# bluenote-1577/sylph

Hardware: AMD Instinct MI355X
Metric: read Gbp/s sketched + genome-comparisons/s profiled, 1 Gbp vs GTDB-R220 (higher is better)
Workload: dtype u64

## Files before the change

sylph_amd/csrc/device_common.h:

```cpp
#pragma once
#include <hip/hip_runtime.h>

#include <cstdint>

#include "seed_plan.h"

namespace sylph {

__device__ __forceinline__ uint64_t mm_hash64(uint64_t key) {
    key = ~(key + (key << 21));
    key = key ^ (key >> 24);
    key = (key + (key << 3)) + (key << 8);
    key = key ^ (key >> 14);
    key = (key + (key << 2)) + (key << 4);
    key = key ^ (key >> 28);
    key = key + (key << 31);
    return key;
}

template <int N>
__device__ __forceinline__ uint64_t lshl_add_u64(uint64_t a, uint64_t b) {
    uint64_t d;
    asm("v_lshl_add_u64 %0, %1, %2, %3" : "=v"(d) : "v"(a), "n"(N), "v"(b));
    return d;
}
template <uint32_t C>
__device__ __forceinline__ uint64_t mul_const_u64(uint64_t t) {
    uint32_t th;
    asm("v_mul_lo_u32 %0, %1, %2" : "=v"(th) : "v"((uint32_t)(t >> 32)), "s"(C));
    uint64_t d, carry;
    asm("v_mad_u64_u32 %0, %1, %2, %3, %4" : "=v"(d), "=s"(carry) : "v"((uint32_t)t), "s"(C - 1u), "v"(((uint64_t)th << 32) | (uint32_t)t));
    return d;
}
__device__ __forceinline__ uint64_t mm_hash64_gfx950(uint64_t key) {
    uint64_t t = lshl_add_u64<0>(key << 21, key);
    {
        uint64_t sh;
        asm("v_lshrrev_b64 %0, 24, %1" : "=v"(sh) : "v"(t));
        uint32_t hi;
        asm("v_bitop3_b32 %0, %1, %2, %3 bitop3:0x96" : "=v"(hi) : "v"((uint32_t)(t >> 32)), "v"((uint32_t)(sh >> 32)), "s"(0xFFFFFF00u));
        t = ((uint64_t)hi << 32) | ((uint32_t)t ^ (uint32_t)sh);
    }
    t = mul_const_u64<265>(t);
    t = t ^ (t >> 14);
    t = lshl_add_u64<4>(t, lshl_add_u64<2>(t, t));
    t = t ^ (t >> 28);
    t = lshl_add_u64<0>(t << 31, t);
    return t;
}
__device__ __forceinline__ uint32_t mm_hash64_gfx950_hi1(uint64_t key) {
    uint64_t t = lshl_add_u64<0>(key << 21, key);
    {
        uint64_t sh;
        asm("v_lshrrev_b64 %0, 24, %1" : "=v"(sh) : "v"(t));
        uint32_t hi;
        asm("v_bitop3_b32 %0, %1, %2, %3 bitop3:0x96" : "=v"(hi) : "v"((uint32_t)(t >> 32)), "v"((uint32_t)(sh >> 32)), "s"(0xFFFFFF00u));
        t = ((uint64_t)hi << 32) | ((uint32_t)t ^ (uint32_t)sh);
    }
    t = mul_const_u64<265>(t);
    t = t ^ (t >> 14);
    t = lshl_add_u64<4>(t, lshl_add_u64<2>(t, t));
    t = t ^ (t >> 28);
    return (uint32_t)(t >> 32) + __builtin_amdgcn_alignbit((uint32_t)(t >> 32), (uint32_t)t, 1) + 1u;
}

__device__ __forceinline__ uint64_t min_u62(uint64_t a, uint64_t b) { uint64_t d; asm("v_min_f64 %0, %1, %2" : "=v"(d) : "v"(a), "v"(b)); return d; }

template <int P>
__device__ __forceinline__ uint32_t fword(uint32_t A0, uint32_t A1, uint32_t A2) {
    static_assert(P >= 0 && P <= 64);
    if constexpr (P == 0) return A0;
    else if constexpr (P < 32) return __builtin_amdgcn_alignbit(A0, A1, 32 - P);
    else if constexpr (P == 32) return A1;
    else if constexpr (P < 64) return __builtin_amdgcn_alignbit(A1, A2, 64 - P);
    else return A2;
}
template <int Q>
__device__ __forceinline__ uint32_t rword(uint32_t B0, uint32_t B1, uint32_t B2) {
    static_assert(Q >= 0 && Q <= 64);
    if constexpr (Q == 0) return B0;
    else if constexpr (Q < 32) return __builtin_amdgcn_alignbit(B1, B0, Q);
    else if constexpr (Q == 32) return B1;
    else if constexpr (Q < 64) return __builtin_amdgcn_alignbit(B2, B1, Q - 32);
    else return B2;
}

__device__ __forceinline__ uint32_t byte_to_seq(uint32_t b) {
    const uint32_t u = b & 0xDFu;
    const uint32_t c = ((b >> 1) ^ (b >> 2)) & 3u;
    const bool acgtu = (u == 'A') | (u == 'C') | (u == 'G') | (u == 'T') | (u == 'U');
    return acgtu ? c : (b <= 3u ? b : 0u);
}

__device__ __forceinline__ uint32_t codes4_fast(uint32_t w, uint32_t& bad) {
    const uint32_t c = ((w >> 1) ^ (w >> 2)) & 0x03030303u;
    const uint32_t expect = __builtin_amdgcn_perm(0u, 0x54474341u , c);
    bad |= (w & 0xDFDFDFDFu) ^ expect;
    return c;
}
__device__ __forceinline__ uint32_t codes4_exact(uint32_t w) {
    return byte_to_seq(w & 0xFFu) | (byte_to_seq((w >> 8) & 0xFFu) << 8) | (byte_to_seq((w >> 16) & 0xFFu) << 16) |
           (byte_to_seq(w >> 24) << 24);
}

__device__ __forceinline__ uint32_t nonzero_bytes(uint32_t x) {
    return (((x & 0x7F7F7F7Fu) + 0x7F7F7F7Fu) | x) & 0x80808080u;
}
__device__ __forceinline__ void clear_invalid_codes(uint32_t w, uint32_t d, uint32_t& c, uint32_t& other) {
    const uint32_t inv = nonzero_bytes(d);
    const uint32_t not_u = nonzero_bytes((w & 0xDFDFDFDFu) ^ 0x55555555u), not_small = nonzero_bytes(w & 0xFCFCFCFCu);
    other |= inv & ~(not_u & not_small);
    c &= ~((inv >> 6) | (inv >> 7));
}

__device__ __forceinline__ uint32_t codes4_bitop(uint32_t w, uint32_t& diff) {
    uint32_t c;
    const uint32_t a = w >> 1, b = w >> 2, m = 0x03030303u, up = 0xDFDFDFDFu;
    asm("v_bitop3_b32 %0, %1, %2, %3 bitop3:0x28" : "=v"(c) : "v"(a), "v"(b), "v"(m));
    const uint32_t expect = __builtin_amdgcn_perm(0u, 0x54474341u , c);
    asm("v_bitop3_b32 %0, %1, %2, %3 bitop3:0x6a" : "=v"(diff) : "v"(w), "v"(up), "v"(expect));
    return c;
}
__device__ __forceinline__ uint32_t pack16_fwd(uint4 v) {
    uint32_t d0, d1, d2, d3, bad;
    uint32_t c0 = codes4_bitop(v.x, d0), c1 = codes4_bitop(v.y, d1), c2 = codes4_bitop(v.z, d2), c3 = codes4_bitop(v.w, d3);
    asm("v_or3_b32 %0, %1, %2, %3" : "=v"(bad) : "v"(d0), "v"(d1), "v"(d2));
    asm("v_or_b32 %0, %1, %2" : "=v"(bad) : "v"(bad), "v"(d3));
    if (bad) {
        uint32_t other = 0;
        clear_invalid_codes(v.x, d0, c0, other); clear_invalid_codes(v.y, d1, c1, other);
        clear_invalid_codes(v.z, d2, c2, other); clear_invalid_codes(v.w, d3, c3, other);
        if (other) { c0 = codes4_exact(v.x); c1 = codes4_exact(v.y); c2 = codes4_exact(v.z); c3 = codes4_exact(v.w); }
    }
    constexpr uint32_t GATHER = (1u << 30) | (1u << 20) | (1u << 10) | 1u;
    const uint32_t p0 = c0 * GATHER, p1 = c1 * GATHER, p2 = c2 * GATHER, p3 = c3 * GATHER;
    return __builtin_amdgcn_perm(p0, p1, 0x07030C0Cu) | __builtin_amdgcn_perm(p2, p3, 0x0C0C0703u);
}

__device__ __forceinline__ uint32_t rcword(uint32_t a) {
    const uint32_t r = __brev(a);
    return ~(((r & 0x55555555u) << 1) | ((r >> 1) & 0x55555555u));
}

__device__ __forceinline__ void pack16(uint4 v, uint32_t& F, uint32_t& R) {
    F = pack16_fwd(v);
    R = rcword(F);
}

using seed_plan::emission_rank;
using seed_plan::n_hashed_kmers;

__device__ __forceinline__ void wave_count_add(unsigned int* counter, bool pred) {
    const unsigned long long m = __ballot(pred);
    if (m && (__lane_id() == (unsigned)__ffsll((long long)m) - 1)) atomicAdd(counter, (unsigned int)__popcll(m));
}

__device__ __forceinline__ uint64_t find_record(const uint64_t* __restrict__ off, uint64_t n, uint64_t p) {
    uint64_t lo = 0, hi = n;
    while (hi - lo > 1) {
        const uint64_t mid = (lo + hi) >> 1;
        if (off[mid] <= p) lo = mid; else hi = mid;
    }
    return lo;
}

__device__ __forceinline__ uint32_t wave_inclusive_sum(uint32_t x) {
    x += (uint32_t)__builtin_amdgcn_update_dpp(0, (int)x, 0x111, 0xF, 0xF, false);
    x += (uint32_t)__builtin_amdgcn_update_dpp(0, (int)x, 0x112, 0xF, 0xF, false);
    x += (uint32_t)__builtin_amdgcn_update_dpp(0, (int)x, 0x114, 0xF, 0xF, false);
    x += (uint32_t)__builtin_amdgcn_update_dpp(0, (int)x, 0x118, 0xF, 0xF, false);
    x += (uint32_t)__builtin_amdgcn_update_dpp(0, (int)x, 0x142, 0xA, 0xF, false);
    x += (uint32_t)__builtin_amdgcn_update_dpp(0, (int)x, 0x143, 0xC, 0xF, false);
    return x;
}

__device__ __forceinline__ uint32_t wave_max_u32(uint32_t x) {
    x = max(x, (uint32_t)__builtin_amdgcn_update_dpp(0, (int)x, 0x111, 0xF, 0xF, false));
    x = max(x, (uint32_t)__builtin_amdgcn_update_dpp(0, (int)x, 0x112, 0xF, 0xF, false));
    x = max(x, (uint32_t)__builtin_amdgcn_update_dpp(0, (int)x, 0x114, 0xF, 0xF, false));
    x = max(x, (uint32_t)__builtin_amdgcn_update_dpp(0, (int)x, 0x118, 0xF, 0xF, false));
    x = max(x, (uint32_t)__builtin_amdgcn_update_dpp(0, (int)x, 0x142, 0xA, 0xF, false));
    x = max(x, (uint32_t)__builtin_amdgcn_update_dpp(0, (int)x, 0x143, 0xC, 0xF, false));
    return (uint32_t)__builtin_amdgcn_readlane((int)x, 63);
}

template <int TPB>
__device__ __forceinline__ uint32_t block_excl_sum(uint32_t v, uint32_t* s_wave, uint32_t* total) {
    const uint32_t lane = threadIdx.x & 63, wave = threadIdx.x >> 6;
    const uint32_t x = wave_inclusive_sum(v);
    __syncthreads();
    if (lane == 63) s_wave[wave] = x;
    __syncthreads();
    uint32_t base = 0, tot = 0;
#pragma unroll
    for (int w = 0; w < TPB / 64; w++) {
        const uint32_t t = s_wave[w];
        if ((uint32_t)w < wave) base += t;
        tot += t;
    }
    if (total) *total = tot;
    return base + x - v;
}

}
```

sylph_amd/csrc/position_road.hip:

```cpp
#include <algorithm>

#include "common.h"
#include "device_common.h"
#include "position_road.h"
#include "seeds.h"

namespace sylph {
namespace {

__device__ __forceinline__ void marker_halves(const uint8_t* __restrict__ p, uint32_t& even, uint32_t& odd) {
    uint32_t e = 0, o = 0;
    uint64_t xs[4];
    __builtin_memcpy(&xs[0], p, 16);
    __builtin_memcpy(&xs[2], p + 16, 16);
#pragma unroll
    for (int w = 0; w < 4; w++) {
        const uint64_t x = xs[w];
        uint32_t bad = 0;
        uint32_t lo = codes4_fast((uint32_t)x, bad), hi = codes4_fast((uint32_t)(x >> 32), bad);
        if (bad) { lo = codes4_exact((uint32_t)x); hi = codes4_exact((uint32_t)(x >> 32)); }
        const uint32_t ev = ((lo & 3u) << 6) | (((lo >> 16) & 3u) << 4) | ((hi & 3u) << 2) | ((hi >> 16) & 3u);
        const uint32_t od = (((lo >> 8) & 3u) << 6) | (((lo >> 24) & 3u) << 4) | (((hi >> 8) & 3u) << 2) | ((hi >> 24) & 3u);
        e = (e << 8) | ev;
        o = (o << 8) | od;
    }
    even = e;
    odd = o;
}

constexpr int COARSE_SHIFT = 14;
__global__ __launch_bounds__(256) void coarse_index_kernel(const uint64_t* __restrict__ off, uint64_t n_rec, uint32_t n_entries,
                                                           uint32_t* __restrict__ coarse) {
    const uint32_t t = blockIdx.x * blockDim.x + threadIdx.x;
    if (t >= n_entries) return;
    const uint64_t total = off[n_rec];
    uint64_t p = (uint64_t)t << COARSE_SHIFT;
    if (total == 0) { coarse[t] = 0; return; }
    if (p >= total) p = total - 1;
    coarse[t] = (uint32_t)find_record(off, n_rec, p);
}

template <bool LIGHT>
__global__ __launch_bounds__(256) void annotate_reads_kernel(
    const uint8_t* __restrict__ bases, const uint64_t* __restrict__ off, uint64_t n_rec, const uint32_t* __restrict__ pos, const uint64_t* __restrict__ hash,
    uint32_t n, uint32_t pos_bias, uint32_t k, int avx2_compat, int paired, int want_markers, uint64_t rec_base, const uint32_t* __restrict__ coarse,
    uint64_t* __restrict__ o_hash, OccRec* __restrict__ o_rec) {
    constexpr uint32_t WIN = 1024;
    __shared__ uint64_t s_lo, s_hi;
    __shared__ uint64_t s_off[WIN + 2];
    const uint32_t first = blockIdx.x * blockDim.x;
    const uint32_t i = first + threadIdx.x;
    const uint64_t total = off[n_rec];
    if (threadIdx.x == 0 || threadIdx.x == 64) {
        const uint32_t j = threadIdx.x == 0 ? first : min(n, first + blockDim.x) - 1;
        uint64_t p = pos[j] >= pos_bias ? pos[j] - pos_bias : 0;
        if (total && p >= total) p = total - 1;
        const uint64_t t = p >> COARSE_SHIFT;
        if (threadIdx.x == 0) s_lo = total ? coarse[t] : 0; else s_hi = (total ? coarse[t + 1] : 0) + 1;
    }
    __syncthreads();
    const uint64_t w_lo = s_lo & ~1ull;
    const uint64_t w_n = min(s_hi + 2, n_rec + 1) - w_lo;
    const bool in_lds = w_n <= WIN + 2;
    if (in_lds)
        for (uint32_t t = threadIdx.x; t < w_n; t += blockDim.x) s_off[t] = off[w_lo + t];
    __syncthreads();
    const bool live = i < n && pos[i] >= pos_bias;
    const uint64_t p = live ? pos[i] - pos_bias : ~0ull;
    uint64_t h = live ? hash[i] : 0, rid = 0, m0 = 0, m1 = 0;
    bool valid = false;
    if (p < total) {
        uint64_t r, start, L, s1 = 0, s2 = 0, e2 = 0;
        auto locate = [&](auto OFF) {
            uint64_t lo = s_lo, hi = s_hi;
            while (hi - lo > 1) {
                const uint64_t mid = (lo + hi) >> 1;
                if (OFF(mid) <= p) lo = mid; else hi = mid;
            }
            r = lo;
            start = OFF(r);
            L = OFF(r + 1) - start;
            if (paired) { const uint64_t r1 = r & ~1ull; s1 = OFF(r1); s2 = OFF(r1 + 1); e2 = OFF(r1 + 2); }
        };
        if (in_lds) locate([&](uint64_t q) -> uint64_t { return s_off[q - w_lo]; });
        else locate([&](uint64_t q) -> uint64_t { return off[q]; });
        valid = (p - start) < n_hashed_kmers(L, k, avx2_compat, 0);
        if (valid) {
            rid = rec_base + r;
            if (!LIGHT && want_markers) {
                const uint8_t* a = nullptr;
                const uint8_t* b = nullptr;
                if (!paired) {
                    if (L >= 66 && L <= 400) { a = bases + start; b = a + L / 2; }
                } else {
                    if (s2 - s1 >= 33 && e2 - s2 >= 33) { a = bases + s1; b = bases + s2; }
                }
                if (a) {
                    uint32_t f, g, rr, t;
                    marker_halves(a, f, g);
                    marker_halves(b, rr, t);
                    m0 = (uint64_t)f | ((uint64_t)rr << 32);
                    m1 = (uint64_t)g | ((uint64_t)t << 32);
                    rid |= RID_MARKER_BIT;
                    if (paired)
                        rid |= min(emission_rank((uint32_t)(p - start), (uint32_t)n_hashed_kmers(L, k, avx2_compat, 0), avx2_compat), RID_RANK_MAX)
                               << RID_RANK_SHIFT;
                }
            }
        }
    }
    if (i < n) {
        const uint64_t hv = valid ? h : INVALID_HASH;
        o_hash[i] = hv;
        if constexpr (!LIGHT) o_rec[i] = OccRec{hv, rid, m0, m1};
    }
}

__global__ __launch_bounds__(256) void annotate_contigs_kernel(const uint64_t* __restrict__ off, uint64_t n_contigs, const uint32_t* __restrict__ pos,
                                                               const uint64_t* __restrict__ hash, uint32_t n, uint32_t k, int avx2_compat,
                                                               uint32_t* __restrict__ o_contig, uint64_t* __restrict__ o_pos, uint64_t* __restrict__ o_hash) {
    const uint32_t i = blockIdx.x * blockDim.x + threadIdx.x;
    if (i >= n) return;
    const uint64_t p = pos[i];
    uint64_t h = INVALID_HASH, endpos = 0;
    uint32_t contig = 0;
    if (p < off[n_contigs]) {
        const uint64_t r = find_record(off, n_contigs, p);
        const uint64_t start = off[r], L = off[r + 1] - start;
        if ((p - start) < n_hashed_kmers(L, k, avx2_compat, 1)) {
            h = hash[i];
            contig = (uint32_t)r;
            endpos = p - start + k - 1;
        }
    }
    o_contig[i] = contig;
    o_pos[i] = endpos;
    o_hash[i] = h;
}

}

PosSeeds seeds_sorted_by_pos(sylph_ctx* ctx, const uint8_t* d_bases, uint64_t n_bases, uint32_t c, uint32_t k, uint32_t* d_count) {
    SY_REQUIRE(n_bases < (1ull << 32), "a batch may hold at most 2^32-1 bases (got %llu)", (unsigned long long)n_bases);
    const PosSeeds none{nullptr, nullptr, 0};
    if (n_bases == 0) return none;
    DevBuf &b_pos = ctx->scratch[2], &b_hash = ctx->scratch[3];
    if (ctx->seeds_mode != 1) {
        HostPhase ph(ctx, "push: seeds (ordered slots)");
        const uint32_t n_tiles = seeds_n_tiles(n_bases), slot_cap = seeds_slot_capacity(c);
        DevBuf &b_sh = ctx->scratch[0], &b_sp = ctx->scratch[1], &b_tc = ctx->scratch[4];
        b_sh.reserve((size_t)n_tiles * slot_cap * 8);
        b_sp.reserve((size_t)n_tiles * slot_cap * 4);
        b_tc.reserve(((size_t)n_tiles + 1) * 4 * 3 + sizeof(SpillState) + 16);
        uint32_t* tile_count = b_tc.as<uint32_t>();
        uint32_t* tile_off = tile_count + (n_tiles + 1);
        uint32_t* spill_slot = tile_off + (n_tiles + 1);
        SpillState* d_spill = reinterpret_cast<SpillState*>(spill_slot + n_tiles + 1);
        SY_HIP(hipMemsetAsync(tile_count + n_tiles, 0, 4, ctx->stream));
        SY_HIP(hipMemsetAsync(d_spill, 0, 4, ctx->stream));
        launch_seeds_slots(ctx, d_bases, (uint32_t)n_bases, c, k, slot_cap, b_sh.as<uint64_t>(), b_sp.as<uint32_t>(), tile_count, d_spill, nullptr, 0, nullptr);
        exclusive_sum_u32(ctx, tile_count, tile_off, (size_t)n_tiles + 1);
        uint32_t res[2] = {0, 0};
        SY_HIP(hipMemcpyAsync(ctx->pinned, tile_off + n_tiles, 4, hipMemcpyDeviceToHost, ctx->stream));
        SY_HIP(hipMemcpyAsync((uint8_t*)ctx->pinned + 4, d_spill, 4, hipMemcpyDeviceToHost, ctx->stream));
        SY_HIP(hipStreamSynchronize(ctx->stream));
        memcpy(res, ctx->pinned, 8);
        if (!ctx->pending.empty()) profile_collect(ctx);
        if (res[1] <= SPILL_MAX_TILES) {
            if (res[0] == 0) return none;
            uint64_t* xh = nullptr;
            uint32_t* xp = nullptr;
            if (res[1]) {
                DevBuf& b_x = ctx->scratch[7];
                const size_t tb = seeds_tile_bases();
                b_x.reserve((size_t)res[1] * tb * 12);
                xh = b_x.as<uint64_t>();
                xp = reinterpret_cast<uint32_t*>(xh + (size_t)res[1] * tb);
                ScopedKernelTimer ts(ctx, "seeds_spill");
                launch_seeds_slots(ctx, d_bases, (uint32_t)n_bases, c, k, slot_cap, xh, xp, tile_count, d_spill, d_spill->tiles, res[1], spill_slot);
            }
            b_pos.reserve((size_t)res[0] * 4);
            b_hash.reserve((size_t)res[0] * 8);
            launch_compact_slots(ctx, b_sh.as<uint64_t>(), b_sp.as<uint32_t>(), tile_count, tile_off, n_tiles, slot_cap, xh, xp, spill_slot,
                                 b_pos.as<uint32_t>(), b_hash.as<uint64_t>());
            return PosSeeds{b_pos.as<uint32_t>(), b_hash.as<uint64_t>(), res[0]};
        }
    }
    uint64_t cap = n_bases / c + n_bases / (4ull * c) + 65536;
    if (cap > n_bases) cap = n_bases;
    uint32_t n = 0;
    for (int attempt = 0; attempt < 2; attempt++) {
        HostPhase ph(ctx, "push: seeds kernel");
        ctx->scratch[0].reserve(cap * 8);
        ctx->scratch[1].reserve(cap * 4);
        static const bool slowlog = getenv("SYLPH_HIP_SLOWLOG") != nullptr;
        const double t0 = slowlog ? HostPhase::now() : 0;
        SY_HIP(hipMemsetAsync(d_count, 0, 4, ctx->stream));
        const double t1 = slowlog ? HostPhase::now() : 0;
        if (slowlog && t1 - t0 > 3.0) fprintf(stderr, "[sylph_hip] slow memset issue %.3f ms\n", t1 - t0);
        launch_seeds(ctx, d_bases, (uint32_t)n_bases, c, k, ctx->scratch[0].as<uint64_t>(), ctx->scratch[1].as<uint32_t>(), (uint32_t)cap, d_count);
        ctx->read_back(&n, d_count, 4);
        if (n <= cap) break;
        cap = n;
        SY_REQUIRE(attempt == 0, "seed buffer overflow persisted");
    }
    if (n == 0) return none;
    HostPhase ph(ctx, "push: sort by position");
    b_pos.reserve((size_t)n * 4);
    b_hash.reserve((size_t)n * 8);
    sort_pairs_u32_u64(ctx, ctx->scratch[1].as<uint32_t>(), b_pos.as<uint32_t>(), ctx->scratch[0].as<uint64_t>(), b_hash.as<uint64_t>(), n, 0,
                       std::max(1, bit_length(n_bases)));
    return PosSeeds{b_pos.as<uint32_t>(), b_hash.as<uint64_t>(), n};
}

void annotate_reads(sylph_sketch* sk, const uint8_t* d_bases, const uint64_t* d_off, uint64_t n_records, uint64_t n_bases, uint32_t bias,
                    const PosSeeds& s, bool plain) {
    sylph_ctx* ctx = sk->ctx;
    const uint32_t n_coarse = (uint32_t)(n_bases >> COARSE_SHIFT) + 2;
    DevBuf& b_coarse = ctx->scratch[5];
    b_coarse.reserve((size_t)n_coarse * 4);
    ScopedKernelTimer t(ctx, "annotate");
    hipLaunchKernelGGL(coarse_index_kernel, dim3(grid_for64(n_coarse)), dim3(256), 0, ctx->stream, d_off, n_records, n_coarse, b_coarse.as<uint32_t>());
    auto annotate = [&](auto kernel, int want_markers, OccRec* o_rec) {
        hipLaunchKernelGGL(kernel, dim3(grid_for64(s.n)), dim3(256), 0, ctx->stream, d_bases, d_off, n_records, s.pos, s.hash, s.n, bias, sk->k, sk->avx2_compat,
                           sk->paired, want_markers, sk->rec_base, b_coarse.as<uint32_t>(), sk->hash.as<uint64_t>() + sk->n_occ, o_rec);
    };
    if (plain) annotate(annotate_reads_kernel<true>, 0, nullptr);
    else annotate(annotate_reads_kernel<false>, sk->no_dedup ? 0 : 1, sk->recs.as<OccRec>() + sk->n_occ);
    SY_HIP(hipGetLastError());
}


struct ContigSeeds { std::vector<uint32_t> contig; std::vector<uint64_t> pos, hash; };

static void seeds_positions_impl(sylph_ctx* ctx, const uint8_t* bases, const uint64_t* contig_off, uint64_t n_contigs, uint32_t c, uint32_t k, int seed_mode, ContigSeeds& out) {
    SY_REQUIRE(c >= 1, "c must be >= 1");
    SY_REQUIRE(seed_mode == SYLPH_SEED_SCALAR || seed_mode == SYLPH_SEED_AVX2_COMPAT, "bad seed_mode %d", seed_mode);
    SY_REQUIRE(k == 21 || k == 31, "k must be 21 or 31 (avx2_seeding.rs:46-52)");
    if (n_contigs == 0) return;
    SY_REQUIRE(contig_off && contig_off[0] == 0, "bad contig offsets");
    SY_REQUIRE(bases || contig_off[n_contigs] == 0, "null bases");
    SY_REQUIRE(n_contigs < (1ull << 32), "too many contigs");
    std::lock_guard<std::mutex> lock(ctx->mu);
    DeviceGuard dg(ctx->device);
    const uint64_t n_bases = contig_off[n_contigs];
    SY_REQUIRE(n_bases < (1ull << 32), "genome larger than 2^32-1 bases: split by contig");
    DevBuf d_bases(ctx), d_off(ctx);
    d_bases.reserve(n_bases + 64);
    d_off.reserve((n_contigs + 1) * 8);
    ctx->h2d(d_bases.p, bases, n_bases);
    ctx->h2d(d_off.p, contig_off, (n_contigs + 1) * 8);
    ctx->counters.reserve(64);
    const PosSeeds s = seeds_sorted_by_pos(ctx, d_bases.as<uint8_t>(), n_bases, c, k, ctx->counters.as<uint32_t>());
    const uint32_t n = s.n;
    if (!n) return;
    DevBuf o_contig(ctx), o_pos(ctx), o_hash(ctx);
    o_contig.reserve((size_t)n * 4);
    o_pos.reserve((size_t)n * 8);
    o_hash.reserve((size_t)n * 8);
    {
        ScopedKernelTimer t(ctx, "annotate");
        hipLaunchKernelGGL(annotate_contigs_kernel, dim3(grid_for64(n)), dim3(256), 0, ctx->stream, d_off.as<uint64_t>(), n_contigs, s.pos, s.hash, n, k,
                           seed_mode == SYLPH_SEED_AVX2_COMPAT, o_contig.as<uint32_t>(), o_pos.as<uint64_t>(), o_hash.as<uint64_t>());
        SY_HIP(hipGetLastError());
    }
    std::vector<uint32_t> hc(n);
    std::vector<uint64_t> hp(n), hh(n);
    ctx->d2h(hc.data(), o_contig.p, (size_t)n * 4);
    ctx->d2h(hp.data(), o_pos.p, (size_t)n * 8);
    ctx->d2h(hh.data(), o_hash.p, (size_t)n * 8);
    out.contig.reserve(n); out.pos.reserve(n); out.hash.reserve(n);
    for (uint32_t i = 0; i < n; i++) {
        if (hh[i] == INVALID_HASH) continue;
        out.contig.push_back(hc[i]); out.pos.push_back(hp[i]); out.hash.push_back(hh[i]);
    }
}

template <class T>
static T* to_malloc(const std::vector<T>& v) {
    T* p = (T*)malloc(std::max<size_t>(1, v.size()) * sizeof(T));
    if (!p) throw std::bad_alloc();
    if (!v.empty()) memcpy(p, v.data(), v.size() * sizeof(T));
    return p;
}

}

using namespace sylph;

extern "C" {

int sylph_seeds_positions(sylph_ctx* ctx, const uint8_t* bases, const uint64_t* contig_off, uint64_t n_contigs, uint32_t c,
                          uint32_t k, int seed_mode, uint32_t** out_contig, uint64_t** out_pos, uint64_t** out_hash,
                          uint64_t* out_n) {
    return guarded([&] {
        SY_REQUIRE(ctx && out_contig && out_pos && out_hash && out_n, "null argument");
        ContigSeeds s;
        seeds_positions_impl(ctx, bases, contig_off, n_contigs, c, k, seed_mode, s);
        *out_contig = to_malloc(s.contig);
        *out_pos = to_malloc(s.pos);
        *out_hash = to_malloc(s.hash);
        *out_n = s.hash.size();
    });
}

int sylph_seeds(sylph_ctx* ctx, const uint8_t* bases, uint64_t len, uint32_t c, uint32_t k, int seed_mode,
                uint64_t** out_hashes, uint64_t* out_n) {
    return guarded([&] {
        SY_REQUIRE(ctx && out_hashes && out_n, "null argument");
        SY_REQUIRE(c >= 1, "c must be >= 1");
        SY_REQUIRE(k == 21 || k == 31, "k must be 21 or 31 (avx2_seeding.rs:46-52)");
        SY_REQUIRE(seed_mode == SYLPH_SEED_SCALAR || seed_mode == SYLPH_SEED_AVX2_COMPAT, "bad seed_mode %d", seed_mode);
        std::vector<uint64_t> res;
        if (len) {
            SY_REQUIRE(bases, "null bases");
            SY_REQUIRE(len < (1ull << 32), "sequence longer than 2^32-1 bases");
            std::lock_guard<std::mutex> lock(ctx->mu);
            DeviceGuard dg(ctx->device);
            DevBuf d_bases(ctx);
            d_bases.reserve(len + 64);
            ctx->h2d(d_bases.p, bases, len);
            ctx->counters.reserve(64);
            const PosSeeds s = seeds_sorted_by_pos(ctx, d_bases.as<uint8_t>(), len, c, k, ctx->counters.as<uint32_t>());
            if (const uint32_t n = s.n) {
                std::vector<uint32_t> hp(n);
                std::vector<uint64_t> hh(n);
                ctx->d2h(hp.data(), s.pos, (size_t)n * 4);
                ctx->d2h(hh.data(), s.hash, (size_t)n * 8);
                const uint64_t nk = n_hashed_kmers(len, k, seed_mode == SYLPH_SEED_AVX2_COMPAT, 0);
                for (uint32_t i = 0; i < n; i++)
                    if (hp[i] < nk) res.push_back(hh[i]);
            }
        }
        *out_hashes = to_malloc(res);
        *out_n = res.size();
    });
}

}
```

sylph_amd/csrc/reads_block.h:

```cpp
#pragma once
#include "common.h"
#include "device_common.h"
#include "seed_plan.h"
#include "sketch_session.h"

namespace sylph {
namespace {

using namespace seed_plan;

template <int K>
struct KC {
    static constexpr uint64_t MASK = (1ull << (2 * K)) - 1;
};

#define SY_LDS __attribute__((address_space(3)))
template <int TPB>
struct ReadsLds {
    SY_LDS uint32_t* sF;
    SY_LDS uint64_t* off;
    SY_LDS uint64_t *m0, *m1;
    SY_LDS uint32_t (*mask)[TPB];
    SY_LDS uint32_t* wave;
    SY_LDS uint32_t* first;
    SY_LDS uint32_t* hist;
    SY_LDS uint32_t* rel;
    SY_LDS uint16_t *perm, *nh;
    SY_LDS uint32_t *redo, *redo_deal;
};
template <int TPB>
__device__ __forceinline__ ReadsLds<TPB> reads_lds() {
    constexpr int OFFS = offs_staged(TPB);
    extern __shared__ uint32_t sF[];
    __shared__ uint64_t s_off[OFFS + 4];
    __shared__ uint32_t s_mask[MASKW][TPB];
    __shared__ uint32_t s_wave[TPB / 64];
    __shared__ uint32_t s_first[TPB + 1], s_rel[TPB];
    __shared__ uint16_t s_perm[TPB], s_nh[TPB];
    __shared__ uint32_t s_redo, s_redo_deal;
    static_assert((OFFS + 4) >= 2 * TPB, "the marker arrays alias the staged offsets");
    static_assert(TPB + 1 >= 64, "the histogram aliases s_first");
    using W = SY_LDS uint32_t*; using D = SY_LDS uint64_t*; using H = SY_LDS uint16_t*;
    return ReadsLds<TPB>{(W)sF, (D)s_off, (D)s_off, (D)s_off + TPB, (SY_LDS uint32_t(*)[TPB])s_mask, (W)s_wave, (W)s_first, (W)s_first, (W)s_rel,
                         (H)s_perm, (H)s_nh, (W)&s_redo, (W)&s_redo_deal};
}

__device__ __forceinline__ uint64_t win64(const SY_LDS uint32_t* sF, uint32_t b) {
    const uint32_t j = b >> 4, ph = (b & 15u) * 2u;
    const uint64_t x = ((uint64_t)sF[j] << 32) | sF[j + 1];
    return (x << ph) | ((uint64_t)sF[j + 2] >> (32u - ph));
}

template <int K>
__device__ __forceinline__ uint64_t revcomp_top(uint64_t x) {
    const uint64_t rev = __brevll(x);
    const uint64_t y = ((rev & 0x5555555555555555ull) << 1) | ((rev >> 1) & 0x5555555555555555ull);
    return (~y) & KC<K>::MASK;
}

__device__ __forceinline__ uint32_t even_fields_to_bytes31(uint32_t w) {
    uint32_t t = w & 0xCCCCCCCCu;
    t = (t | (t << 2)) & 0xF0F0F0F0u;
    return t | (t << 4);
}
__device__ __forceinline__ void evenodd16(uint64_t x, uint32_t& ev, uint32_t& od) {
    const uint32_t hi = (uint32_t)(x >> 32), lo = (uint32_t)x;
    ev = __builtin_amdgcn_perm(even_fields_to_bytes31(hi), even_fields_to_bytes31(lo), 0x07050301u);
    od = __builtin_amdgcn_perm(even_fields_to_bytes31(hi << 2), even_fields_to_bytes31(lo << 2), 0x07050301u);
}

struct HitRegs {
    uint32_t bit[16];
    uint32_t zero;
    uint64_t exec0;
};
__device__ __forceinline__ HitRegs hit_regs() {
    HitRegs r;
#pragma unroll
    for (int t = 0; t < 16; t++) asm("v_mov_b32 %0, %1" : "=v"(r.bit[t]) : "s"(hit_const(t)));
    asm("v_mov_b32 %0, 0" : "=v"(r.zero));
    r.exec0 = 0;
    return r;
}
__device__ __forceinline__ void hit_clear_lower(uint32_t& addr, uint32_t zero) { asm("ds_write_b16 %0, %1" : "+v"(addr) : "v"(zero)); }
__device__ __forceinline__ void hit_chain_begin(uint32_t& addr) { asm volatile("" : "+v"(addr) : : "memory"); }
__device__ __forceinline__ void hit_chain_end(uint32_t& addr) { asm volatile("s_waitcnt lgkmcnt(0)" : "+v"(addr) : : "memory"); }

template <int K, int T, int HV, bool LB>
__device__ __forceinline__ void kmer_step(uint32_t A0, uint32_t A1, uint32_t A2, uint32_t B0, uint32_t B1, uint32_t B2,
                                          uint64_t thr, uint32_t& mask, const HitRegs& hit) {
    static_assert(2 * K <= 62 && 2 * K > 32, "min_u62 wants both windows below 2^62; the high word holds 2K - 32 bits");
    constexpr int HB = 2 * K - 32, T0 = T & ~1;
    uint32_t fhi, rhi;
    if constexpr (2 * T + HB <= 32) {
        fhi = __builtin_amdgcn_ubfe(A0, 32 - HB - 2 * T, HB); rhi = __builtin_amdgcn_ubfe(B1, 2 * T, HB);
    } else {
        const uint32_t cf = fword<2 * T0>(A0, A1, A2), cr = rword<2 * T0 + 32>(B0, B1, B2);
        fhi = __builtin_amdgcn_ubfe(cf, 32 - HB - 2 * (T - T0), HB); rhi = __builtin_amdgcn_ubfe(cr, 2 * (T - T0), HB);
    }
    const uint32_t flo = fword<2 * T + HB>(A0, A1, A2), rlo = rword<2 * T>(B0, B1, B2);
    const uint64_t canon = min_u62(((uint64_t)fhi << 32) | flo, ((uint64_t)rhi << 32) | rlo);
    if constexpr (HV == 2) {
        const uint32_t u = mm_hash64_gfx950_hi1(canon);
        if constexpr (LB)
            asm("v_cmpx_ge_u32 vcc, %2, %1\n\tds_xor_b32 %0, %3\n\ts_mov_b64 exec, %4"
                : "+v"(mask) : "v"(u), "s"((uint32_t)thr), "v"(hit.bit[T]), "s"(hit.exec0) : "vcc");
        else
            asm("v_cmp_ge_u32 vcc, %2, %1\n\tv_addc_co_u32 %0, vcc, %0, %0, vcc" : "+v"(mask) : "v"(u), "s"((uint32_t)thr) : "vcc");
    } else {
        const uint64_t h = HV ? mm_hash64_gfx950(canon) : mm_hash64(canon);
        if constexpr (LB)
            asm("v_cmpx_lt_u64 vcc, %1, %2\n\tds_xor_b32 %0, %3\n\ts_mov_b64 exec, %4"
                : "+v"(mask) : "v"(h), "s"(thr), "v"(hit.bit[T]), "s"(hit.exec0) : "vcc");
        else
            asm("v_cmp_lt_u64 vcc, %1, %2\n\tv_addc_co_u32 %0, vcc, %0, %0, vcc" : "+v"(mask) : "v"(h), "s"(thr) : "vcc");
    }
}
template <int K, int T0, int HV, bool LB>
__device__ __forceinline__ void kmer_steps8(uint32_t A0, uint32_t A1, uint32_t A2, uint32_t B0, uint32_t B1, uint32_t B2,
                                            uint64_t thr, uint32_t& mask, const HitRegs& hit) {
    kmer_step<K, T0 + 0, HV, LB>(A0, A1, A2, B0, B1, B2, thr, mask, hit);
    kmer_step<K, T0 + 1, HV, LB>(A0, A1, A2, B0, B1, B2, thr, mask, hit);
    kmer_step<K, T0 + 2, HV, LB>(A0, A1, A2, B0, B1, B2, thr, mask, hit);
    kmer_step<K, T0 + 3, HV, LB>(A0, A1, A2, B0, B1, B2, thr, mask, hit);
    kmer_step<K, T0 + 4, HV, LB>(A0, A1, A2, B0, B1, B2, thr, mask, hit);
    kmer_step<K, T0 + 5, HV, LB>(A0, A1, A2, B0, B1, B2, thr, mask, hit);
    kmer_step<K, T0 + 6, HV, LB>(A0, A1, A2, B0, B1, B2, thr, mask, hit);
    kmer_step<K, T0 + 7, HV, LB>(A0, A1, A2, B0, B1, B2, thr, mask, hit);
}

template <int ENC, int TPB>
__device__ __forceinline__ void load_stream(SY_LDS uint32_t* sF, const uint8_t* bases_al, uint64_t n_al, uint32_t blk, int64_t a0, uint32_t n_words) {
    const uint32_t tid = threadIdx.x;
    const bool interior = block_starts_inside(blk) && (uint64_t)(a0 + (int64_t)n_words * 16) <= n_al;
    const uintptr_t src0 = (uintptr_t)bases_al + (uintptr_t)(ENC == 0 ? a0 : (a0 >> 2));
    constexpr uint32_t WB = ENC == 0 ? 16u : 4u;
    if (interior) {
        if constexpr (ENC == 0) {
            for (uint32_t ci = tid; ci < n_words; ci += TPB) sF[ci] = pack16_fwd(*reinterpret_cast<const uint4*>(src0 + ci * WB));
        } else {
            for (uint32_t ci = tid; ci < n_words; ci += TPB)
                sF[ci] = __builtin_amdgcn_perm(0u, *reinterpret_cast<const uint32_t*>(src0 + ci * WB), 0x00010203u);
        }
    } else {
        uint32_t ci_lo, ci_hi;
        stream_word_range(a0, n_al, n_words, ci_lo, ci_hi);
        for (uint32_t ci = tid; ci < n_words; ci += TPB) {
            const bool inside = ci >= ci_lo && ci < ci_hi;
            if constexpr (ENC == 0) {
                uint4 v = make_uint4(0, 0, 0, 0);
                if (inside) v = *reinterpret_cast<const uint4*>(src0 + ci * WB);
                sF[ci] = pack16_fwd(v);
            } else {
                uint32_t w = 0;
                if (inside) w = *reinterpret_cast<const uint32_t*>(src0 + ci * WB);
                sF[ci] = __builtin_amdgcn_perm(0u, w, 0x00010203u);
            }
        }
    }
}

template <int TPB>
__device__ __forceinline__ bool stage_offsets(const ReadsLds<TPB> s, const uint64_t* off, uint64_t n_rec, uint32_t R0, uint32_t R1,
                                              uint32_t w_lo) {
    const uint32_t w_hi = R1 + min((uint32_t)n_rec - R1, 2u);
    const uint32_t n_stage = w_hi - w_lo + 1;
    const bool in_lds = n_stage <= (uint32_t)(offs_staged(TPB) + 4) && (R1 - R0) <= (uint32_t)TPB;
    if (in_lds) {
        const uint64_t* const src = off + w_lo;
        for (uint32_t t = threadIdx.x; t < n_stage; t += TPB) s.off[t] = src[t];
    }
    return in_lds;
}

template <int K, int TPB>
__device__ __forceinline__ bool record_geometry(const ReadsLds<TPB> s, const uint64_t* off, bool in_lds, uint32_t w_lo, uint32_t r,
                                                bool active, int paired, uint32_t rb, int avx2_compat, int want_markers, uint32_t& nh,
                                                uint32_t& rel, uint32_t& ba, uint32_t& bb) {
    uint64_t o0 = 0, o1 = 0, o2 = 0;
    if (active) {
        const uint32_t r0 = paired ? (r & ~1u) : r;
        if (in_lds) {
            const SY_LDS uint64_t* const o = s.off + (r0 - w_lo);
            o0 = o[0]; o1 = o[1];
            if (paired) o2 = o[2];
        } else {
            const uint64_t* const o = off + r0;
            o0 = o[0]; o1 = o[1];
            if (paired) o2 = o[2];
        }
    }
    const uint64_t d1 = o1 - o0, d2 = o2 - o1;
    const bool too_long = d1 > (uint64_t)RH || (paired && d2 > (uint64_t)RH);
    const bool mate2 = paired && (r & 1u);
    const uint32_t L = too_long ? 0u : (uint32_t)(mate2 ? d2 : d1);
    const uint32_t rel1 = record_rel32(o0, rb), rel2 = record_rel32(o1, rb);
    nh = (uint32_t)n_hashed_kmers(L, K, avx2_compat, 0);
    rel = active ? (mate2 ? rel2 : rel1) : 0u;
    MarkerBases mk{0u, 0u};
    if (want_markers && active && !too_long) mk = paired ? pair_marker_bases(rel1, rel2, (uint32_t)d1, (uint32_t)d2) : single_marker_bases(rel, L);
    ba = mk.ba; bb = mk.bb;
    return too_long;
}

template <int TPB, bool LB>
__device__ __forceinline__ bool deal_by_length(const ReadsLds<TPB> s, uint32_t nh, uint32_t rel, uint32_t& slot, uint32_t& rel_h, uint32_t& nh_h,
                                               uint32_t& rows) {
    const uint32_t tid = threadIdx.x, lane = tid & 63;
    if (tid < 64) s.hist[tid] = 0;
    s.rel[tid] = rel;
    s.nh[tid] = (uint16_t)nh;
    if (tid == 0) *s.redo_deal = 0;
    __syncthreads();
    if (__ballot(nh != (uint32_t)s.nh[0]) && lane == 0) *s.redo_deal = 1;
    __syncthreads();
    const bool dealt = *s.redo_deal != 0;
    const uint32_t bin = deal_bin(nh);
    uint32_t hg_max = half_groups(nh), arrival = 0, hc = 0;
    if (dealt) {
        arrival = atomicAdd((uint32_t*)&s.hist[bin], 1u);
        __syncthreads();
        hc = s.hist[lane];
        const uint64_t bins_used = __ballot(hc != 0u);
        hg_max = bins_used ? 63u - (uint32_t)(__ffsll((unsigned long long)bins_used) - 1) : 0u;
    }
    rows = rows_used(hg_max);
    if constexpr (LB) {
        const uint32_t rows_u = (uint32_t)__builtin_amdgcn_readfirstlane((int)rows);
        for (uint32_t w = 0; w < rows_u; w += 2) { s.mask[w][tid] = 0; s.mask[w + 1][tid] = 0; }
    }
    if (dealt) {
        const uint32_t incl = wave_inclusive_sum(hc);
        s.perm[(uint32_t)__shfl((int)(incl - hc), (int)bin) + arrival] = (uint16_t)tid;
        __syncthreads();
    }
    slot = dealt ? s.perm[tid] : tid;
    rel_h = dealt ? s.rel[slot] : rel;
    nh_h = dealt ? s.nh[slot] : nh;
    return dealt;
}

template <int K, int HV, int TPB, bool LB>
__device__ __forceinline__ void hash_record(const ReadsLds<TPB> s, uint32_t slot, uint32_t rel_h, uint32_t nh_h, uint64_t thr_loop,
                                            const HitRegs& hit_consts) {
    const SY_LDS uint32_t* const sF = s.sF;
    const uint32_t nh_max = wave_max_u32(nh_h);
    if (nh_max) {
        const uint32_t w0 = rel_h >> 4, sh = 32u - (rel_h & 15u) * 2u;
        uint32_t raw = sF[w0], nxt = sF[w0 + 1];
        auto next_word = [&](uint32_t j) {
            const uint32_t a = (uint32_t)((((uint64_t)raw << 32) | nxt) >> sh);
            raw = nxt;
            nxt = sF[w0 + j + 2];
            return a;
        };
        uint32_t A0 = next_word(0), A1 = next_word(1), A2 = next_word(2);
        uint32_t B0 = rcword(A0), B1 = rcword(A1), B2 = rcword(A2);
        const uint32_t n_half = half_groups(nh_max);
        SY_LDS uint16_t* const mask_half = (SY_LDS uint16_t*)&s.mask[0][slot];
        const uint32_t n_grp = n_half >> 1;
        if constexpr (LB) {
            HitRegs hit = hit_consts;
            hit.exec0 = __builtin_amdgcn_read_exec();
            uint32_t addr = (uint32_t)(uintptr_t)&s.mask[0][slot];
            hit_chain_begin(addr);
            for (uint32_t g = 0; g < n_grp; g++) {
                kmer_steps8<K, 0, HV, true>(A0, A1, A2, B0, B1, B2, thr_loop, addr, hit);
                kmer_steps8<K, 8, HV, true>(A0, A1, A2, B0, B1, B2, thr_loop, addr, hit);
                A0 = A1; A1 = A2; A2 = next_word(g + 3);
                B0 = B1; B1 = B2; B2 = rcword(A2);
                if (hit_clear_after(g)) hit_clear_lower(addr, hit.zero);
                else addr += hit_word_offset(2, TPB);
            }
            if (n_half & 1u) {
                kmer_steps8<K, 0, HV, true>(A0, A1, A2, B0, B1, B2, thr_loop, addr, hit);
                if (hit_clear_after(n_grp)) hit_clear_lower(addr, hit.zero);
            }
            hit_chain_end(addr);
            return;
        }
        const HitRegs hit{};
        for (uint32_t g = 0; g < n_grp; g++) {
            uint32_t mask = 0;
            kmer_steps8<K, 0, HV, false>(A0, A1, A2, B0, B1, B2, thr_loop, mask, hit);
            kmer_steps8<K, 8, HV, false>(A0, A1, A2, B0, B1, B2, thr_loop, mask, hit);
            A0 = A1; A1 = A2; A2 = next_word(g + 3);
            B0 = B1; B1 = B2; B2 = rcword(A2);
            mask_half[group_half(g, TPB)] = (uint16_t)mask;
        }
        if (n_half & 1u) {
            uint32_t mask = 0;
            kmer_steps8<K, 0, HV, false>(A0, A1, A2, B0, B1, B2, thr_loop, mask, hit);
            mask_half[group_half(n_grp, TPB)] = (uint16_t)(mask << 8);
        }
    }
}

template <int TPB>
__device__ __forceinline__ uint32_t count_hits(const ReadsLds<TPB> s, uint32_t nh, bool decode, uint32_t& first, uint32_t& total) {
    const uint32_t tid = threadIdx.x;
    uint32_t cnt = 0;
    const uint32_t nw = mask_words(nh);
    for (uint32_t w = 0; w + 1 < nw; w++) {
        uint32_t m = s.mask[w][tid];
        if (decode) { m = hit_decode(m); s.mask[w][tid] = m; }
        cnt += __popc(m);
    }
    if (nw) {
        const uint32_t m0 = s.mask[nw - 1][tid];
        const uint32_t m = (decode ? hit_decode(m0) : m0) & tail_mask(nh);
        s.mask[nw - 1][tid] = m;
        cnt += __popc(m);
    }
    first = block_excl_sum<TPB>(cnt, (uint32_t*)s.wave, &total);
    return cnt;
}

template <int TPB>
__device__ __forceinline__ void publish_markers(const ReadsLds<TPB> s, uint32_t cnt, uint32_t first, uint32_t total, uint32_t ba, uint32_t bb) {
    const uint32_t tid = threadIdx.x;
    uint64_t m0 = 0, m1 = 0;
    const uint32_t has = (cnt && bb) ? 1u : 0u;
    if (has) {
        const uint64_t wa64 = win64(s.sF, ba), wb64 = win64(s.sF, bb);
        uint32_t ea, oa, eb, ob;
        evenodd16(wa64, ea, oa);
        evenodd16(wb64, eb, ob);
        m0 = (uint64_t)ea | ((uint64_t)eb << 32);
        m1 = (uint64_t)oa | ((uint64_t)ob << 32);
    }
    s.m0[tid] = m0;
    s.m1[tid] = m1;
    s.first[tid] = first | (has << 31);
    if (tid == 0) s.first[TPB] = total;
}

template <int TPB>
__device__ __forceinline__ bool list_survivors(const ReadsLds<TPB> s, uint32_t nh, uint32_t cnt, uint32_t first, uint32_t total, uint32_t rows) {
    const uint32_t tid = threadIdx.x;
    SY_LDS uint32_t* const s_owner = &s.mask[0][0] + rows * TPB;
    const bool is_listed = listed(total, rows, TPB);
    if (is_listed && cnt) {
        uint32_t p = first;
        for (uint32_t w = 0; w < mask_words(nh); w++) {
            uint32_t m = s.mask[w][tid];
            while (m) {
                const uint32_t bpos = (uint32_t)__clz((int)m);
                s_owner[p++] = tid | ((w * 32 + bpos) << OWNER_LANE_BITS);
                m &= ~(0x80000000u >> bpos);
            }
        }
    }
    return is_listed;
}

template <int K, int HV, int TPB>
__device__ __forceinline__ void finish_survivors(const ReadsLds<TPB> s, bool is_listed, uint32_t rows, uint32_t total, uint32_t base_prev,
                                                 uint32_t slot_cap, uint64_t thr, uint64_t rec_base, uint64_t pass, int paired, int avx2_compat,
                                                 uint64_t out0, OccRec* slot_rec, uint32_t* slot_key, int key_sh) {
    const SY_LDS uint32_t* const s_owner = &s.mask[0][0] + rows * TPB;
    for (uint32_t hix = threadIdx.x; hix < total; hix += TPB) {
        uint32_t lo, i = 0, f;
        if (is_listed) {
            const uint32_t ow = s_owner[hix];
            lo = ow & ((1u << OWNER_LANE_BITS) - 1u);
            i = ow >> OWNER_LANE_BITS;
            f = s.first[lo];
        } else {
            lo = 0;
            uint32_t hi = TPB;
            while (hi - lo > 1) {
                const uint32_t mid = (lo + hi) >> 1;
                if ((s.first[mid] & 0x7FFFFFFFu) <= hix) lo = mid; else hi = mid;
            }
            f = s.first[lo];
            uint32_t j = hix - (f & 0x7FFFFFFFu);
            for (uint32_t w = 0; w < MASKW; w++) {
                uint32_t m = s.mask[w][lo];
                const uint32_t c = (uint32_t)__popc(m);
                if (j >= c) { j -= c; continue; }
                for (; j; j--) m &= ~(0x80000000u >> __clz((int)m));
                i = w * 32 + (uint32_t)__clz((int)m);
                break;
            }
        }
        const uint32_t o = base_prev + hix;
        if (o < slot_cap) {
            const uint64_t ft = win64(s.sF, s.rel[lo] + i);
            const uint64_t fk = ft >> (64 - 2 * K), rk = revcomp_top<K>(ft);
            const uint64_t h = mm_hash64_gfx950(fk < rk ? fk : rk);
            if constexpr (HV == 2) {
                if (h >= thr) {
                    atomicAnd((uint32_t*)&s.mask[kmer_word(i)][lo], ~(1u << kmer_bit(i)));
                    *s.redo = 1u;
                    continue;
                }
            }
            uint64_t rid = rec_base + pass + lo;
            if (f >> 31) {
                rid |= RID_MARKER_BIT;
                if (paired) rid |= min(emission_rank(i, s.nh[lo], avx2_compat), RID_RANK_MAX) << RID_RANK_SHIFT;
            }
            slot_rec[out0 + o] = OccRec{h, rid, s.m0[lo], s.m1[lo]};
            if (slot_key) slot_key[out0 + o] = (uint32_t)(h >> key_sh);
        }
    }
}

#undef SY_LDS

}
}
```

Before: 1248.

## Replace nucleotide decode with byte-permute lookup table and restructure stream loading

```diff
diff --git a/sylph_amd/csrc/device_common.h b/sylph_amd/csrc/device_common.h
--- a/sylph_amd/csrc/device_common.h
+++ b/sylph_amd/csrc/device_common.h
@@ -3,6 +3,7 @@
 
 #include <cstdint>
 
+#include "pack_plan.h"
 #include "seed_plan.h"
 
 namespace sylph {
@@ -85,56 +86,28 @@
     else return B2;
 }
 
-__device__ __forceinline__ uint32_t byte_to_seq(uint32_t b) {
-    const uint32_t u = b & 0xDFu;
-    const uint32_t c = ((b >> 1) ^ (b >> 2)) & 3u;
-    const bool acgtu = (u == 'A') | (u == 'C') | (u == 'G') | (u == 'T') | (u == 'U');
-    return acgtu ? c : (b <= 3u ? b : 0u);
-}
+using pack_plan::byte_to_seq;
+using pack_plan::codes4_exact;
 
-__device__ __forceinline__ uint32_t codes4_fast(uint32_t w, uint32_t& bad) {
-    const uint32_t c = ((w >> 1) ^ (w >> 2)) & 0x03030303u;
-    const uint32_t expect = __builtin_amdgcn_perm(0u, 0x54474341u , c);
-    bad |= (w & 0xDFDFDFDFu) ^ expect;
-    return c;
-}
-__device__ __forceinline__ uint32_t codes4_exact(uint32_t w) {
-    return byte_to_seq(w & 0xFFu) | (byte_to_seq((w >> 8) & 0xFFu) << 8) | (byte_to_seq((w >> 16) & 0xFFu) << 16) |
-           (byte_to_seq(w >> 24) << 24);
-}
-
-__device__ __forceinline__ uint32_t nonzero_bytes(uint32_t x) {
-    return (((x & 0x7F7F7F7Fu) + 0x7F7F7F7Fu) | x) & 0x80808080u;
-}
-__device__ __forceinline__ void clear_invalid_codes(uint32_t w, uint32_t d, uint32_t& c, uint32_t& other) {
-    const uint32_t inv = nonzero_bytes(d);
-    const uint32_t not_u = nonzero_bytes((w & 0xDFDFDFDFu) ^ 0x55555555u), not_small = nonzero_bytes(w & 0xFCFCFCFCu);
-    other |= inv & ~(not_u & not_small);
-    c &= ~((inv >> 6) | (inv >> 7));
-}
-
-__device__ __forceinline__ uint32_t codes4_bitop(uint32_t w, uint32_t& diff) {
-    uint32_t c;
-    const uint32_t a = w >> 1, b = w >> 2, m = 0x03030303u, up = 0xDFDFDFDFu;
-    asm("v_bitop3_b32 %0, %1, %2, %3 bitop3:0x28" : "=v"(c) : "v"(a), "v"(b), "v"(m));
-    const uint32_t expect = __builtin_amdgcn_perm(0u, 0x54474341u , c);
-    asm("v_bitop3_b32 %0, %1, %2, %3 bitop3:0x6a" : "=v"(diff) : "v"(w), "v"(up), "v"(expect));
-    return c;
+__device__ __forceinline__ uint32_t codes4_table(uint32_t w) {
+    const uint32_t e = __builtin_amdgcn_perm(pack_plan::TAB_HI, pack_plan::TAB_LO, w & pack_plan::LOW3);
+    uint32_t t;
+    asm("v_bitop3_b32 %0, %1, %2, %3 bitop3:0x6a" : "=v"(t) : "v"(w), "s"(pack_plan::UPPER), "v"(e));
+    return t;
 }
 __device__ __forceinline__ uint32_t pack16_fwd(uint4 v) {
-    uint32_t d0, d1, d2, d3, bad;
-    uint32_t c0 = codes4_bitop(v.x, d0), c1 = codes4_bitop(v.y, d1), c2 = codes4_bitop(v.z, d2), c3 = codes4_bitop(v.w, d3);
-    asm("v_or3_b32 %0, %1, %2, %3" : "=v"(bad) : "v"(d0), "v"(d1), "v"(d2));
-    asm("v_or_b32 %0, %1, %2" : "=v"(bad) : "v"(bad), "v"(d3));
+    uint32_t t0 = codes4_table(v.x), t1 = codes4_table(v.y), t2 = codes4_table(v.z), t3 = codes4_table(v.w), any, bad;
+    asm("v_or3_b32 %0, %1, %2, %3" : "=v"(any) : "v"(t0), "v"(t1), "v"(t2));
+    asm("v_bitop3_b32 %0, %1, %2, %3 bitop3:0xa8" : "=v"(bad) : "v"(any), "v"(t3), "s"(pack_plan::ODD));
     if (bad) {
-        uint32_t other = 0;
-        clear_invalid_codes(v.x, d0, c0, other); clear_invalid_codes(v.y, d1, c1, other);
-        clear_invalid_codes(v.z, d2, c2, other); clear_invalid_codes(v.w, d3, c3, other);
-        if (other) { c0 = codes4_exact(v.x); c1 = codes4_exact(v.y); c2 = codes4_exact(v.z); c3 = codes4_exact(v.w); }
+        t0 = pack_plan::clear_odd_codes(t0); t1 = pack_plan::clear_odd_codes(t1);
+        t2 = pack_plan::clear_odd_codes(t2); t3 = pack_plan::clear_odd_codes(t3);
+        if (pack_plan::row_has_raw_small(v.x, v.y, v.z, v.w)) {
+            t0 = codes4_exact(v.x); t1 = codes4_exact(v.y); t2 = codes4_exact(v.z); t3 = codes4_exact(v.w);
+        }
     }
-    constexpr uint32_t GATHER = (1u << 30) | (1u << 20) | (1u << 10) | 1u;
-    const uint32_t p0 = c0 * GATHER, p1 = c1 * GATHER, p2 = c2 * GATHER, p3 = c3 * GATHER;
-    return __builtin_amdgcn_perm(p0, p1, 0x07030C0Cu) | __builtin_amdgcn_perm(p2, p3, 0x0C0C0703u);
+    const uint32_t p0 = t0 * pack_plan::GATHER, p1 = t1 * pack_plan::GATHER, p2 = t2 * pack_plan::GATHER, p3 = t3 * pack_plan::GATHER;
+    return __builtin_amdgcn_perm(p0, p1, pack_plan::GATHER_SEL_01) | __builtin_amdgcn_perm(p2, p3, pack_plan::GATHER_SEL_23);
 }
 
 __device__ __forceinline__ uint32_t rcword(uint32_t a) {
diff --git a/sylph_amd/csrc/pack_plan.h b/sylph_amd/csrc/pack_plan.h
--- /dev/null
+++ b/sylph_amd/csrc/pack_plan.h
@@ -0,0 +1,102 @@
+#pragma once
+#include <cstdint>
+
+#if defined(__HIPCC__)
+#define SY_PACK_HD __host__ __device__ __forceinline__
+#else
+#define SY_PACK_HD inline
+#endif
+
+namespace sylph {
+namespace pack_plan {
+
+SY_PACK_HD constexpr uint32_t byte_to_seq(uint32_t b) {
+    const uint32_t u = b & 0xDFu;
+    const uint32_t c = ((b >> 1) ^ (b >> 2)) & 3u;
+    const bool acgtu = (u == 'A') | (u == 'C') | (u == 'G') | (u == 'T') | (u == 'U');
+    return acgtu ? c : (b <= 3u ? b : 0u);
+}
+
+constexpr uint32_t N_LETTERS = 5;
+constexpr uint8_t LETTER[N_LETTERS] = {'A', 'C', 'G', 'T', 'U'};
+constexpr uint8_t LETTER_CODE[N_LETTERS] = {0, 1, 2, 3, 3};
+constexpr uint32_t table_entry(uint32_t i) {
+    for (uint32_t l = 0; l < N_LETTERS; l++)
+        if ((LETTER[l] & 7u) == i) return (uint32_t)(LETTER[l] ^ LETTER_CODE[l]);
+    return 0xFFu;
+}
+constexpr uint32_t table_word(uint32_t i0) {
+    return table_entry(i0) | (table_entry(i0 + 1) << 8) | (table_entry(i0 + 2) << 16) | (table_entry(i0 + 3) << 24);
+}
+constexpr uint32_t TAB_LO = table_word(0), TAB_HI = table_word(4);
+constexpr uint32_t LOW3 = 0x07070707u;
+constexpr uint32_t UPPER = 0xDFDFDFDFu;
+constexpr uint32_t ODD = 0xF8F8F8F8u;
+static_assert(TAB_LO == 0x42FF41FFu && TAB_HI == 0x45FF5657u, "E = {FF, 41, FF, 42, 57, 56, FF, 45}");
+static_assert((ODD & 0xFFu) == (0xFFu & ~7u) && ODD == (ODD & 0xFFu) * 0x01010101u, "the row test's mask covers exactly bits 7:3 of every byte");
+constexpr bool letters_fit_table() {
+    for (uint32_t l = 0; l < N_LETTERS; l++) {
+        for (uint32_t m = 0; m < l; m++) if ((LETTER[l] & 7u) == (LETTER[m] & 7u)) return false;
+        if (table_entry(LETTER[l] & 7u) != (uint32_t)(LETTER[l] ^ LETTER_CODE[l])) return false;
+        if ((LETTER[l] & 0x20u) || LETTER_CODE[l] > 3u || byte_to_seq(LETTER[l]) != LETTER_CODE[l]) return false;
+    }
+    return true;
+}
+static_assert(letters_fit_table(), "the table entries follow from the five letters and their codes");
+
+constexpr uint32_t perm_b32(uint32_t hi, uint32_t lo, uint32_t sel) {
+    const uint64_t src = ((uint64_t)hi << 32) | lo;
+    uint32_t d = 0;
+    for (int j = 0; j < 4; j++) {
+        const uint32_t s = (sel >> (8 * j)) & 0xFFu;
+        const uint32_t byte = s < 8u ? (uint32_t)(src >> (8 * s)) & 0xFFu : 0u;
+        d |= byte << (8 * j);
+    }
+    return d;
+}
+
+constexpr uint32_t codes4_table(uint32_t w) {
+    const uint32_t e = perm_b32(TAB_HI, TAB_LO, w & LOW3);
+    return (w & UPPER) ^ e;
+}
+constexpr bool table_matches_rule() {
+    for (uint32_t b = 0; b < 256; b++) {
+        const uint32_t t = codes4_table(b * 0x01010101u) & 0xFFu, u = b & 0xDFu;
+        const bool letter = u == 'A' || u == 'C' || u == 'G' || u == 'T' || u == 'U';
+        if (letter ? t != byte_to_seq(b) : (t & ODD) == 0u) return false;
+    }
+    return true;
+}
+static_assert(table_matches_rule(), "t is the code for the ten letters and has a bit of 7:3 set for the 246 other bytes");
+
+SY_PACK_HD constexpr uint32_t odd_bytes(uint32_t t) {
+    const uint32_t y = ((t & ODD) >> 3) + 0x7F7F7F7Fu;
+    return ((y >> 7) & 0x01010101u) * 0xFFu;
+}
+SY_PACK_HD constexpr uint32_t clear_odd_codes(uint32_t t) { return t & ~odd_bytes(t); }
+SY_PACK_HD constexpr uint32_t not_raw_small(uint32_t w) { return ((w >> 2) & 0x3F3F3F3Fu) + 0x7F7F7F7Fu; }
+SY_PACK_HD constexpr bool row_has_raw_small(uint32_t w0, uint32_t w1, uint32_t w2, uint32_t w3) {
+    return (not_raw_small(w0) & not_raw_small(w1) & not_raw_small(w2) & not_raw_small(w3) & 0x80808080u) != 0x80808080u;
+}
+SY_PACK_HD constexpr uint32_t codes4_exact(uint32_t w) {
+    return byte_to_seq(w & 0xFFu) | (byte_to_seq((w >> 8) & 0xFFu) << 8) | (byte_to_seq((w >> 16) & 0xFFu) << 16) |
+           (byte_to_seq(w >> 24) << 24);
+}
+
+constexpr uint32_t GATHER = (1u << 30) | (1u << 20) | (1u << 10) | 1u;
+constexpr uint32_t GATHER_SEL_01 = 0x07030C0Cu, GATHER_SEL_23 = 0x0C0C0703u;
+constexpr uint32_t row_is_odd(uint32_t t0, uint32_t t1, uint32_t t2, uint32_t t3) { return (t0 | t1 | t2 | t3) & ODD; }
+constexpr uint32_t pack16_fwd(uint32_t w0, uint32_t w1, uint32_t w2, uint32_t w3) {
+    uint32_t t0 = codes4_table(w0), t1 = codes4_table(w1), t2 = codes4_table(w2), t3 = codes4_table(w3);
+    if (row_is_odd(t0, t1, t2, t3)) {
+        t0 = clear_odd_codes(t0); t1 = clear_odd_codes(t1); t2 = clear_odd_codes(t2); t3 = clear_odd_codes(t3);
+        if (row_has_raw_small(w0, w1, w2, w3)) {
+            t0 = codes4_exact(w0); t1 = codes4_exact(w1); t2 = codes4_exact(w2); t3 = codes4_exact(w3);
+        }
+    }
+    const uint32_t p0 = t0 * GATHER, p1 = t1 * GATHER, p2 = t2 * GATHER, p3 = t3 * GATHER;
+    return perm_b32(p0, p1, GATHER_SEL_01) | perm_b32(p2, p3, GATHER_SEL_23);
+}
+
+}
+}
diff --git a/sylph_amd/csrc/position_road.hip b/sylph_amd/csrc/position_road.hip
--- a/sylph_amd/csrc/position_road.hip
+++ b/sylph_amd/csrc/position_road.hip
@@ -16,9 +16,8 @@
 #pragma unroll
     for (int w = 0; w < 4; w++) {
         const uint64_t x = xs[w];
-        uint32_t bad = 0;
-        uint32_t lo = codes4_fast((uint32_t)x, bad), hi = codes4_fast((uint32_t)(x >> 32), bad);
-        if (bad) { lo = codes4_exact((uint32_t)x); hi = codes4_exact((uint32_t)(x >> 32)); }
+        uint32_t lo = codes4_table((uint32_t)x), hi = codes4_table((uint32_t)(x >> 32));
+        if ((lo | hi) & pack_plan::ODD) { lo = codes4_exact((uint32_t)x); hi = codes4_exact((uint32_t)(x >> 32)); }
         const uint32_t ev = ((lo & 3u) << 6) | (((lo >> 16) & 3u) << 4) | ((hi & 3u) << 2) | ((hi >> 16) & 3u);
         const uint32_t od = (((lo >> 8) & 3u) << 6) | (((lo >> 24) & 3u) << 4) | (((hi >> 8) & 3u) << 2) | ((hi >> 24) & 3u);
         e = (e << 8) | ev;
diff --git a/sylph_amd/csrc/reads_block.h b/sylph_amd/csrc/reads_block.h
--- a/sylph_amd/csrc/reads_block.h
+++ b/sylph_amd/csrc/reads_block.h
@@ -129,36 +129,48 @@
     kmer_step<K, T0 + 7, HV, LB>(A0, A1, A2, B0, B1, B2, thr, mask, hit);
 }
 
+#define SY_GLOBAL __attribute__((address_space(1)))
+template <int ENC>
+struct StreamRow;
+template <>
+struct StreamRow<0> {
+    using In = uint32_t __attribute__((ext_vector_type(4)));
+    static __device__ __forceinline__ In zero() { return In{0, 0, 0, 0}; }
+    static __device__ __forceinline__ uint32_t word(In v) { return pack16_fwd(make_uint4(v.x, v.y, v.z, v.w)); }
+};
+template <>
+struct StreamRow<1> {
+    using In = uint32_t;
+    static __device__ __forceinline__ In zero() { return 0u; }
+    static __device__ __forceinline__ uint32_t word(In w) { return __builtin_amdgcn_perm(0u, w, 0x00010203u); }
+};
 template <int ENC, int TPB>
 __device__ __forceinline__ void load_stream(SY_LDS uint32_t* sF, const uint8_t* bases_al, uint64_t n_al, uint32_t blk, int64_t a0, uint32_t n_words) {
+    using Row = StreamRow<ENC>;
+    using In = typename Row::In;
     const uint32_t tid = threadIdx.x;
     const bool interior = block_starts_inside(blk) && (uint64_t)(a0 + (int64_t)n_words * 16) <= n_al;
-    const uintptr_t src0 = (uintptr_t)bases_al + (uintptr_t)(ENC == 0 ? a0 : (a0 >> 2));
-    constexpr uint32_t WB = ENC == 0 ? 16u : 4u;
+    const SY_GLOBAL In* src = reinterpret_cast<const SY_GLOBAL In*>((uintptr_t)bases_al + (uintptr_t)(ENC == 0 ? a0 : (a0 >> 2)));
     if (interior) {
-        if constexpr (ENC == 0) {
-            for (uint32_t ci = tid; ci < n_words; ci += TPB) sF[ci] = pack16_fwd(*reinterpret_cast<const uint4*>(src0 + ci * WB));
-        } else {
-            for (uint32_t ci = tid; ci < n_words; ci += TPB)
-                sF[ci] = __builtin_amdgcn_perm(0u, *reinterpret_cast<const uint32_t*>(src0 + ci * WB), 0x00010203u);
-        }
+        SY_LDS uint32_t* dst = sF + tid;
+        auto row = [&] {
+            uint32_t lane_off = tid * (uint32_t)sizeof(In);
+            asm volatile("" : "+v"(lane_off));
+            return Row::word(*reinterpret_cast<const SY_GLOBAL In*>(reinterpret_cast<const SY_GLOBAL uint8_t*>(src) + lane_off));
+        };
+        for (uint32_t rows = n_words / TPB; rows; rows--, src += TPB, dst += TPB) *dst = row();
+        if (tid < n_words % TPB) *dst = row();
     } else {
         uint32_t ci_lo, ci_hi;
         stream_word_range(a0, n_al, n_words, ci_lo, ci_hi);
         for (uint32_t ci = tid; ci < n_words; ci += TPB) {
-            const bool inside = ci >= ci_lo && ci < ci_hi;
-            if constexpr (ENC == 0) {
-                uint4 v = make_uint4(0, 0, 0, 0);
-                if (inside) v = *reinterpret_cast<const uint4*>(src0 + ci * WB);
-                sF[ci] = pack16_fwd(v);
-            } else {
-                uint32_t w = 0;
-                if (inside) w = *reinterpret_cast<const uint32_t*>(src0 + ci * WB);
-                sF[ci] = __builtin_amdgcn_perm(0u, w, 0x00010203u);
-            }
-        }
-    }
-}
+            In v = Row::zero();
+            if (ci >= ci_lo && ci < ci_hi) v = src[ci];
+            sF[ci] = Row::word(v);
+        }
+    }
+}
+#undef SY_GLOBAL
 
 template <int TPB>
 __device__ __forceinline__ bool stage_offsets(const ReadsLds<TPB> s, const uint64_t* off, uint64_t n_rec, uint32_t R0, uint32_t R1,
```

Measured after the change: 1258, median of 6. No clear change (+0.8%).
